# volume-em/empanada

Measured on AMD Instinct MI355X. Metric: Mvox/s end-to-end 3D panoptic inference (incl. consensus); PQ vs CPU ref, higher is better.
Workload: dtype f32

## Files before the change

### empanada_amd/_hip.py

```python
import ctypes
import os

import torch

_HERE = os.path.dirname(os.path.abspath(__file__))
LIB_PATH = os.path.join(_HERE, 'libemp_hip.so')

MAX_KS = 11
MAX_CLASSES = 16
MAX_CENTERS = 4096
CENTER_LIMIT = 65535


class HipError(RuntimeError):
    pass


_c = ctypes
_P = _c.c_void_p
_I = _c.c_int
_L = _c.c_int64
_F = _c.c_float
_U32 = _c.c_uint32

SIGNATURES = {
    'emp_version': (_I, []),
    'emp_last_error': (_c.c_char_p, []),
    'emp_device_count': (_I, []),
    'emp_bn_act_nhwc': (_I, [_P, _P, _P, _P, _I, _L, _I, _P, _L, _P]),
    'emp_dwconv_nhwc': (_I, [_P, _P, _P, _I, _I, _I, _I, _I, _P, _P]),
    'emp_upsample_bilinear': (_I, [_P, _I, _I, _I, _I, _P, _P, _I, _I, _P, _P]),
    'emp_conv_bn_act_proj_nhwc': (_I, [_P, _P, _P, _P, _I] + [_I] * 10 + [_P, _I, _P, _P, _L, _P]),
    'emp_conv_k_slab': (_I, [_L, _I, _I, _I]),
    'emp_conv_k_slab_cin': (_I, [_L, _I, _I, _I, _I]),
    'emp_conv_k_slab_geom': (_I, [_L, _I, _I, _I, _I, _I, _I, _I, _I]),
    'emp_conv1x1_ws_eligible': (_I, [_L, _I, _I, _I, _I, _I, _I, _I]),
    'emp_conv1x1_ws_kind_for': (_I, [_L, _I, _I, _I, _I, _I, _I, _I, _I]),
    'emp_conv1x1_ws_launches': (_L, [_I]),
    'emp_gconv_chunk': (_I, [_I]),
    'emp_gconv3x3_bn_act_nhwc': (_I, [_P, _L, _P, _P, _P, _I, _I, _I, _I, _I, _I, _I, _P, _L, _P]),
    'emp_conv_bn_act_nhwc': (_I, [_P, _P, _P, _P, _P, _L, _I] + [_I] * 10 + [_P, _L, _P]),
    'emp_conv_splitk_plan': (_I, [_L, _I, _I, _I, _I]),
    'emp_conv_splitk_bn_act_nhwc': (_I, [_P, _P, _P, _P, _P, _L, _I] + [_I] * 11 + [_P, _P, _L, _P]),
    'emp_wino_input_transform': (_I, [_P, _I, _I, _I, _I, _I, _P, _L, _P, _P]),
    'emp_gemm_nt_batched': (_I, [_P, _P, _I, _L, _I, _I, _P, _P]),
    'emp_wino4_input_transform': (_I, [_P, _I, _I, _I, _I, _I, _P, _L, _P, _P]),
    'emp_wino4_output_transform': (_I, [_P, _P, _L, _I, _I, _I, _I, _I, _P, _P, _I, _P, _L, _P]),
    'emp_wino4_conv_bn_act_nhwc': (_I, [_P, _I, _I, _I, _I, _I, _P, _L, _P, _I, _P, _P, _I, _P, _L, _P]),
    'emp_wino4_fused_eligible': (_I, [_L, _I, _I, _I]),
    'emp_wino3_input_transform': (_I, [_P, _I, _I, _I, _I, _I, _P, _L, _P, _P]),
    'emp_wino3_output_transform': (_I, [_P, _P, _L, _I, _I, _I, _I, _I, _P, _P, _I, _P, _L, _P]),
    'emp_wino_gemm_fused': (_I, [_P, _I, _I, _I, _I, _I, _P, _L, _P, _I, _P, _P]),
    'emp_wino_output_transform': (_I, [_P, _P, _L, _I, _I, _I, _I, _I, _P, _P, _I, _P, _L, _P]),
    'emp_chain_class': (_I, [_L, _P, _P, _P, _I, _P, _P, _P, _P, _L, _L, _c.c_double, _c.c_double, _P, _P, _P, _P]),
    'emp_lsap_maximize': (_L, [_P, _L, _L, _P, _P]),
    'emp_slices_to_input': (_I, [_P, _L, _L, _L, _I, _I, _I, _I, _I, _F, _F, _P, _P]),
    'emp_slices_to_input_scaled': (_I, [_P, _L, _L, _L] + [_I] * 7 + [_P, _P, _P, _P, _I, _F, _F, _P, _P]),
    'emp_pointwise_out_nhwc': (_I, [_P, _P, _P, _L, _L, _I, _I, _P, _P]),
    'emp_bn_relu_maxpool_nhwc': (_I, [_P, _P, _P, _I, _I, _I, _I, _P, _P]),
    'emp_stem_conv7_bn_relu_maxpool': (_I, [_P, _P, _P, _P, _I, _I, _I, _P, _P]),
    'emp_logits_to_prob': (_I, [_P, _I, _I, _L, _P, _P]),
    'emp_upsample_bilinear_prob': (_I, [_P, _I, _I, _I, _I, _P, _P, _I, _I, _P, _I, _P]),
    'emp_pr_upsample2x': (_I, [_P, _I, _I, _I, _I, _P, _P, _P]),
    'emp_pr_topk_work_bytes': (_L, [_I, _L]),
    'emp_pr_topk': (_I, [_P, _I, _L, _I, _P, _L, _P, _P]),
    'emp_pr_point_sample': (_I, [_P, _L, _P, _I, _I, _I, _I, _I, _P, _I, _I, _I, _P, _P, _I, _P]),
    'emp_pr_scatter': (_I, [_P, _I, _P, _I, _I, _I, _L, _P, _P]),
    'emp_median_harden_stack': (_I, [_P, _I, _I, _L, _I, _F, _P, _P, _P]),
    'emp_median_step': (_I, [_c.POINTER(_P), _I, _L, _P, _P]),
    'emp_harden': (_I, [_P, _I, _I, _L, _F, _P, _P]),
    'emp_find_centers': (_I, [_P, _I, _I, _I, _F, _I, _I, _P, _P, _P]),
    'emp_find_centers_work_elems': (_L, [_I, _I, _I, _I]),
    'emp_find_centers_ws': (_I, [_P, _I, _I, _I, _F, _I, _I, _P, _P, _P, _P]),
    'emp_group_work_elems': (_L, [_I, _I]),
    'emp_group_pixels': (_I, [_P, _P, _I, _P, _I, _I, _I, _I, _P, _U32, _P, _P, _P]),
    'emp_fuse_work_elems': (_L, [_I, _I, _I]),
    'emp_fuse_panoptic': (_I, [_P, _P, _I, _I, _I, _I, _I, _I, _U32, _L, _L, _L, _P, _P, _P, _P]),
    'emp_fuse_lut': (_I, [_P, _P, _I, _I, _I, _I, _I, _I, _U32, _L, _L, _P, _P]),
    'emp_fuse_apply': (_I, [_P, _P, _I, _I, _I, _I, _I, _I, _U32, _L, _L, _P, _P, _P, _P]),
    'emp_runs_count': (_I, [_P, _I, _I, _I, _P, _P]),
    'emp_scan_tmp_elems': (_L, [_L]),
    'emp_exclusive_scan_i32': (_I, [_P, _L, _P, _P, _P]),
    'emp_runs_extract': (_I, [_P, _I, _I, _I, _P, _P, _P, _P, _P]),
    'emp_runs_label_work_elems': (_L, [_L]),
    'emp_runs_label': (_I, [_P, _P, _P, _P, _L, _I, _I, _I, _L, _U32, _P, _P, _P, _P, _P, _P, _P, _P, _P]),
    'emp_runs_overlap_next': (_I, [_P, _P, _P, _P, _P, _L, _I, _I, _I, _L, _P, _L, _P, _P]),
    'emp_rle_decode': (_I, [_P, _P, _P, _L, _P, _P]),
    'emp_rle_encode_work_elems': (_L, [_L]),
    'emp_rle_encode': (_I, [_P, _L, _P, _P, _P, _P, _P]),
    'emp_box_pairs': (_I, [_P, _L, _P, _L, _I, _P, _P, _I, _P, _L, _P, _P]),
    'emp_rle_pair_intersections': (_I, [_P, _P, _P, _P, _L, _P, _P]),
    'emp_sort_work_bytes': (_L, [_L]),
    'emp_sort_u64_i32': (_I, [_P, _P, _P, _P, _L, _I, _I, _P, _L, _P]),
    'emp_vote_work_bytes': (_L, [_L]),
    'emp_vote_ranges': (_I, [_P, _P, _P, _L, _I, _I, _P, _L, _P, _P, _P]),
    'emp_fill_runs_u32': (_I, [_P, _L, _P, _P, _P, _L, _P, _P]),
    'emp_fill_table_u32': (_I, [_P, _L, _I, _I, _P, _P, _P, _P, _P, _L, _P]),
    'emp_scatter_yz_u32': (_I, [_P, _I, _I, _I, _P, _P, _P, _P, _P, _L, _P]),
    'emp_fill_runs_u8': (_I, [_P, _L, _P, _P, _L, _c.c_uint8, _P]),
    'emp_triplets_reduce_work_bytes': (_L, [_L]),
    'emp_triplets_reduce': (_I, [_P, _L, _P, _L, _P, _P, _P]),
    'emp_track_work_elems': (_L, [_L]),
    'emp_track_lift': (_I, [_I, _P, _P, _P, _P, _P, _L, _I, _I, _I, _I, _I, _L, _P, _P, _P, _P, _P]),
    'emp_track_lift_yz': (_I, [_P, _P, _P, _P, _L, _L, _I, _I, _I, _L, _P, _P, _P]),
    'emp_tile_lift': (_I, [_P, _P, _P, _P, _P, _L, _I, _I, _I, _I, _L, _P, _P, _P, _P, _P]),
    'emp_track_sort_work_bytes': (_L, [_L]),
    'emp_track_sort': (_I, [_P, _P, _L, _I, _P, _L, _P, _P, _P, _P, _P]),
    'emp_track_offsets': (_I, [_P, _L, _L, _P, _P]),
    'emp_track_expand': (_I, [_P, _P, _L, _L, _P, _P]),
    'emp_track_clip': (_I, [_P, _P, _L, _L, _L, _P, _P, _P, _P, _P]),
}

_lib = None


def load():
    global _lib
    if _lib is None:
        if not os.path.exists(LIB_PATH):
            raise HipError(f"{LIB_PATH} not found: build it with `python -m empanada_amd.build` "
                           "(hipcc --offload-arch=gfx950). There is no CPU fallback.")
        lib = ctypes.CDLL(LIB_PATH)
        for name, (res, args) in SIGNATURES.items():
            fn = getattr(lib, name)
            fn.restype = res
            fn.argtypes = args
        _lib = lib
    return _lib


def require_gpu():
    if torch.cuda._is_in_bad_fork():
# ... 695 lines not shown
    N, C, h, w = logits.shape
    assert logits.is_cuda and logits.dtype == torch.float32 and logits.is_contiguous()
    up = torch.empty((N, C, 2 * h, 2 * w), dtype=torch.float32, device=logits.device)
    unc = torch.empty((N, 4 * h * w), dtype=torch.float32, device=logits.device)
    call('emp_pr_upsample2x', logits.data_ptr(), N, C, h, w, up.data_ptr(), unc.data_ptr(), stream(),
         alg_bytes=4 * (logits.numel() + up.numel() + unc.numel()))
    return up, unc


def pr_topk(unc, k):
    require_gpu()
    N, HW = unc.shape
    assert unc.is_cuda and unc.dtype == torch.float32 and unc.is_contiguous() and 1 <= k <= HW
    wb = query('emp_pr_topk_work_bytes', N, HW)
    work = torch.empty((wb,), dtype=torch.uint8, device=unc.device)
    idx = torch.empty((N, k), dtype=torch.int32, device=unc.device)
    call('emp_pr_topk', unc.data_ptr(), N, HW, int(k), _ptr(work), wb, _ptr(idx), stream(), alg_bytes=4 * 6 * unc.numel())
    return idx


def pr_point_sample(features, coarse, idx, H, W, ld):
    require_gpu()
    N, CF, Hf, Wf = features.shape
    C = coarse.shape[1]
    assert features.is_cuda and features.dtype == torch.float32 and features.stride(1) == 1
    fps = features.stride(3)
    assert features.stride(2) == Wf * fps and features.stride(0) == Hf * Wf * fps, "NHWC features required"
    assert coarse.is_contiguous() and coarse.shape == (N, C, Hf, Wf) and idx.shape[0] == N and idx.dtype == torch.int32
    k = idx.shape[1]
    X0 = torch.empty((N * k, ld), dtype=torch.float32, device=features.device)
    X1 = torch.empty((N * k, ld), dtype=torch.float32, device=features.device)
    call('emp_pr_point_sample', features.data_ptr(), fps, coarse.data_ptr(), N, Hf, Wf, CF, C, _ptr(idx), k, int(H), int(W),
         X0.data_ptr(), X1.data_ptr(), int(ld), stream(), alg_bytes=4 * N * k * (4 * CF + 2 * ld))
    return X0, X1


def pr_scatter(points, idx, logits):
    require_gpu()
    N, C, H, W = logits.shape
    k = idx.shape[1]
    assert points.shape[0] == N * k and points.stride(1) == 1 and logits.is_contiguous()
    call('emp_pr_scatter', points.data_ptr(), points.stride(0), _ptr(idx), N, C, k, H * W, logits.data_ptr(), stream(),
         alg_bytes=8 * N * k * C)
    return logits


def as_pixels(mat, cols=None):
    P, ld = mat.shape
    v = mat.view(1, P, 1, ld).permute(0, 3, 1, 2)
    return v if cols is None else v[:, :cols]


def stem_conv7_bn_relu_maxpool(x, w_tc, scale, shift):
    require_gpu()
    N, C, H, W = x.shape
    assert C == 1 and x.is_cuda and x.dtype == torch.float32 and x.is_contiguous()
    assert tuple(w_tc.shape) == (49, 64) and w_tc.is_contiguous()
    OH, OW = (H - 1) // 2 + 1, (W - 1) // 2 + 1
    PH, PW = (OH - 1) // 2 + 1, (OW - 1) // 2 + 1
    y = torch.empty((N, 64, PH, PW), dtype=torch.float32, device=x.device, memory_format=torch.channels_last)
    call('emp_stem_conv7_bn_relu_maxpool', x.data_ptr(), _ptr(w_tc), _ptr(scale), _ptr(shift), N, H, W, y.data_ptr(),
         stream(), alg_bytes=4 * (x.numel() + y.numel()), alg_flops=2 * N * OH * OW * 64 * 49)
    return y


def wino4_filter_transform(w_oihw):
    g = w_oihw.detach().double().cpu()

    def comb(a, b, c):
        return [a / 4.0, -((a + b) + c) / 6.0, ((b - a) - c) / 6.0, (a / 24.0 + b / 12.0) + c / 6.0,
                (a / 24.0 - b / 12.0) + c / 6.0, c]

    rows = comb(g[:, :, 0, :], g[:, :, 1, :], g[:, :, 2, :])
    U = []
    for r in rows:
        U.extend(comb(r[:, :, 0], r[:, :, 1], r[:, :, 2]))
    return torch.stack(U, dim=0).float().contiguous()


def wino4_fused_eligible(T, Cin, Cout, has_scale_shift=True):
    return bool(load().emp_wino4_fused_eligible(int(T), int(Cin), int(Cout), int(bool(has_scale_shift))))


def wino4_conv_bn_act(x, U, tiles_dev, dil, scale=None, shift=None, relu=False, out=None, fused=None):
    require_gpu()
    N, Cin, H, W = x.shape
    Cout = U.shape[1]
    assert x.is_cuda and x.dtype == torch.float32 and x.is_contiguous(memory_format=torch.channels_last)
    T = tiles_dev.shape[0]
    if fused is None:
        fused = wino4_fused_eligible(T, Cin, Cout, scale is not None and shift is not None)
    if out is None:
        out = torch.empty((N, Cout, H, W), dtype=torch.float32, device=x.device, memory_format=torch.channels_last)
    assert out.shape == (N, Cout, H, W) and out.stride(1) == 1
    ops = out.stride(3)
    assert out.stride(2) == W * ops and out.stride(0) == H * W * ops, "NHWC channel slice required"
    st = stream()
    if fused:
        call('emp_wino4_conv_bn_act_nhwc', x.data_ptr(), N, H, W, Cin, dil, _ptr(tiles_dev), T, _ptr(U), Cout,
             _ptr(scale), _ptr(shift), int(bool(relu)), out.data_ptr(), ops, st, profile_as='emp_gemm_nt_batched',
             alg_bytes=4 * (x.numel() + U.numel() + N * Cout * H * W), alg_flops=2 * 36 * T * Cout * Cin)
        return out
    V = torch.empty((36, T, Cin), dtype=torch.float32, device=x.device)
    Mw = torch.empty((36, T, Cout), dtype=torch.float32, device=x.device)
    call('emp_wino4_input_transform', x.data_ptr(), N, H, W, Cin, dil, _ptr(tiles_dev), T, _ptr(V), st,
         alg_bytes=4 * (x.numel() + V.numel()))
    call('emp_gemm_nt_batched', _ptr(V), _ptr(U), 36, T, Cout, Cin, _ptr(Mw), st,
         alg_bytes=4 * (V.numel() + U.numel() + Mw.numel()), alg_flops=2 * 36 * T * Cout * Cin)
    call('emp_wino4_output_transform', _ptr(Mw), _ptr(tiles_dev), T, N, H, W, Cout, dil, _ptr(scale), _ptr(shift),
         int(bool(relu)), out.data_ptr(), ops, st, alg_bytes=4 * (Mw.numel() + N * Cout * H * W))
    return out


def conv_k_slab(M, Cout, batch=1, has_residual=False, Cin=None, geom=None, relu=False):
    if geom is not None:
        KH, KW, stride, pad = geom
        return int(load().emp_conv_k_slab_geom(int(M), int(Cout), int(bool(has_residual)), int(Cin), int(KH), int(KW),
                                               int(stride), int(pad), 2 if relu == 'gate' else int(bool(relu))))
    if Cin is not None:
        return int(load().emp_conv_k_slab_cin(int(M), int(Cout), int(batch), int(bool(has_residual)), int(Cin)))
    return int(load().emp_conv_k_slab(int(M), int(Cout), int(batch), int(bool(has_residual))))


_WINO3_G = [[0.5, 0.0, 0.0], [-0.5, -0.5, -0.5], [-1.0 / 6, 1.0 / 6, -1.0 / 6], [1.0 / 6, 1.0 / 3, 2.0 / 3], [0.0, 0.0, 1.0]]


def wino3_filter_transform(w_oihw):
    g = w_oihw.detach().double().cpu()

    def comb(a, b, c):
        return [(G[0] * a + G[1] * b) + G[2] * c for G in _WINO3_G]

    rows = comb(g[:, :, 0, :], g[:, :, 1, :], g[:, :, 2, :])
    U = []
    for r in rows:
        U.extend(comb(r[:, :, 0], r[:, :, 1], r[:, :, 2]))
    return torch.stack(U, dim=0).float().contiguous()


def wino3_conv_bn_act(x, U, tiles_dev, dil, scale=None, shift=None, relu=False, out=None):
    require_gpu()
    N, Cin, H, W = x.shape
    Cout = U.shape[1]
    assert x.is_cuda and x.dtype == torch.float32 and x.is_contiguous(memory_format=torch.channels_last)
    T = tiles_dev.shape[0]
    V = torch.empty((25, T, Cin), dtype=torch.float32, device=x.device)
    Mw = torch.empty((25, T, Cout), dtype=torch.float32, device=x.device)
    if out is None:
        out = torch.empty((N, Cout, H, W), dtype=torch.float32, device=x.device, memory_format=torch.channels_last)
    assert out.shape == (N, Cout, H, W) and out.stride(1) == 1
    ops = out.stride(3)
    assert out.stride(2) == W * ops and out.stride(0) == H * W * ops, "NHWC channel slice required"
    st = stream()
    call('emp_wino3_input_transform', x.data_ptr(), N, H, W, Cin, dil, _ptr(tiles_dev), T, _ptr(V), st,
         alg_bytes=4 * (x.numel() + V.numel()))
    call('emp_gemm_nt_batched', _ptr(V), _ptr(U), 25, T, Cout, Cin, _ptr(Mw), st,
         alg_bytes=4 * (V.numel() + U.numel() + Mw.numel()), alg_flops=2 * 25 * T * Cout * Cin)
    call('emp_wino3_output_transform', _ptr(Mw), _ptr(tiles_dev), T, N, H, W, Cout, dil, _ptr(scale), _ptr(shift),
         int(bool(relu)), out.data_ptr(), ops, st, alg_bytes=4 * (Mw.numel() + N * Cout * H * W))
    return out


def conv_bn_act_proj_nhwc(x, w_okkc, scale, shift, relu, proj_w, proj_b=None, stride=1, pad=0, dil=1, keep=False):
    require_gpu()
    N, Cin, H, W = x.shape
    Cout, KH, KW, _ = w_okkc.shape
# ... 15 lines not shown
```

### empanada_amd/csrc/emp_wino4.hip

```cpp
#include "emp_common.h"
#include "emp_wino4.h"
#include <stdlib.h>
#include <type_traits>

typedef float f32x4 __attribute__((ext_vector_type(4)));

#define WF_THREADS 512
#define WF_G 32
#define WF_S 16
#define WF_RS 34
#define WF_PS (WF_S * WF_RS)
#define WF_PF 3
#define WF_XCH (WF_THREADS * 48)
#define WF_T_MIN 3136

struct WfGeom {
    const float *x, *U, *scale, *shift;
    const int32_t *tiles;
    float *out;
    int64_t T, out_ps;
    int H, W, dil, groups;
};

template <int CIN, int COUT, bool RELU>
__global__ __launch_bounds__(WF_THREADS, 2) void wino4_fused_kernel(WfGeom g)
{
    constexpr int KS = CIN / WF_S;
    constexpr int CG = COUT / 64;
    __shared__ __attribute__((aligned(16))) float Vs[36 * WF_PS > WF_XCH ? 36 * WF_PS : WF_XCH];

    const int tid = threadIdx.x, wave = tid >> 6, lane = tid & 63;
    const int tl = tid >> 4, ch = tid & 15;
    const int ci = lane & 15, q = lane >> 4;
    const int odd = q >> 1;
    const int h = wave >> 2, w4 = wave & 3;

    const int xcd = blockIdx.x & 7, slot = blockIdx.x >> 3, per = gridDim.x >> 3;
    const int lo = (int)((int64_t)g.groups * xcd / 8), hi = (int)((int64_t)g.groups * (xcd + 1) / 8);
    const int n_items = slot < hi - lo ? ((hi - lo - slot + per - 1) / per) * CG : 0;

    auto load_raw = [&](int item, int s, v1 (&raw)[6][6]) -> int {
        const int64_t t = (int64_t)(lo + slot + (item / CG) * per) * WF_G + tl;
        const bool live = t < g.T;
        const int64_t tc = live ? t : g.T - 1;
        const int n = g.tiles[3 * tc], by = g.tiles[3 * tc + 1], bx = g.tiles[3 * tc + 2];
        const uint32_t src = 4u * ((uint32_t)n * (uint32_t)(g.H * g.W * CIN) + (uint32_t)(WF_S * s + ch));
        const char *xb = reinterpret_cast<const char *>(g.x);
        int mask = 0;
        uint32_t xo[6];
#pragma unroll
        for (int b = 0; b < 6; ++b) {
            const int xx = bx + b * g.dil;
            if (live && xx >= 0 && xx < g.W) mask |= 64 << b;
            xo[b] = 4u * (uint32_t)(min(max(xx, 0), g.W - 1) * CIN);
        }
#pragma unroll
        for (int a = 0; a < 6; ++a) {
            const int yy = by + a * g.dil;
            if (live && yy >= 0 && yy < g.H) mask |= 1 << a;
            const uint32_t row = src + 4u * (uint32_t)(min(max(yy, 0), g.H - 1) * (g.W * CIN));
#pragma unroll
            for (int b = 0; b < 6; ++b) raw[a][b] = {*reinterpret_cast<const float *>(xb + (row + xo[b]))};
        }
        return mask;
    };
    auto transform = [&](const v1 (&raw)[6][6], int mask) {
        v1 tt[6][6];
#pragma unroll
        for (int a = 0; a < 6; ++a) {
            v1 d[6];
#pragma unroll
            for (int b = 0; b < 6; ++b) d[b] = {(mask >> a & 1) && (mask >> (6 + b) & 1) ? raw[a][b].x : 0.f};
            wino4_bt(d, tt[a]);
        }
        float *dst = &Vs[ch * WF_RS + tl];
#pragma unroll
        for (int v = 0; v < 6; ++v) {
            v1 col[6], r[6];
#pragma unroll
            for (int a = 0; a < 6; ++a) col[a] = tt[a][v];
            wino4_bt(col, r);
#pragma unroll
            for (int u = 0; u < 6; ++u) dst[(u * 6 + v) * WF_PS] = r[u].x;
        }
    };

    const float *Al = &Vs[3 * h * WF_PS + (8 * (q & 1) + odd) * WF_RS + ci];
    const float *Ul = g.U + ((int64_t)3 * h * COUT + 16 * w4 + ci) * CIN + 8 * (q & 1) + 4 * odd;

    v1 raw[6][6];
    int mask = 0;
    if (n_items > 0) mask = load_raw(0, 0, raw);
    for (int item = 0; item < n_items; ++item) {
        const int cg = item % CG;
        f32x4 acc[18][2];
#pragma unroll
        for (int lp = 0; lp < 18; ++lp)
#pragma unroll
            for (int rt = 0; rt < 2; ++rt) acc[lp][rt] = {0.f, 0.f, 0.f, 0.f};

#pragma unroll 1
        for (int s = 0; s < KS; ++s) {
            transform(raw, mask);
            __syncthreads();
            const float *up = Ul + (int64_t)cg * 64 * CIN + WF_S * s;
            auto uoff = [](int lp) { return (int64_t)((lp / 3) * 6 + lp % 3) * COUT * CIN; };
            float4 bq[WF_PF];
#pragma unroll
            for (int lp = 0; lp < WF_PF; ++lp) bq[lp] = *reinterpret_cast<const float4 *>(up + uoff(lp));
            if (s + 1 < KS) mask = load_raw(item, s + 1, raw);
#pragma unroll
            for (int lp = 0; lp < 18; ++lp) {
                float4 c = bq[lp % WF_PF];
                asm volatile("" : "+v"(c.x), "+v"(c.y), "+v"(c.z), "+v"(c.w));
                if (lp + WF_PF < 18) bq[lp % WF_PF] = *reinterpret_cast<const float4 *>(up + uoff(lp + WF_PF));
                const auto s0 = __builtin_amdgcn_permlane32_swap(__float_as_uint(c.x), __float_as_uint(c.y), false, false);
                const auto s1 = __builtin_amdgcn_permlane32_swap(__float_as_uint(c.z), __float_as_uint(c.w), false, false);
                const float bv[4] = {__uint_as_float(s0[0]), __uint_as_float(s1[0]), __uint_as_float(s0[1]), __uint_as_float(s1[1])};
                const float *ap = Al + ((lp / 3) * 6 + lp % 3) * WF_PS;
#pragma unroll
                for (int j = 0; j < 4; ++j)
#pragma unroll
                    for (int rt = 0; rt < 2; ++rt)
                        acc[lp][rt] = __builtin_amdgcn_mfma_f32_16x16x4f32(ap[2 * j * WF_RS + 16 * rt], bv[j], acc[lp][rt], 0, 0, 0);
            }
            __syncthreads();
        }

        const int co = cg * 64 + 16 * w4 + ci;
        float keep[4][3][4];
        float *xw = &Vs[((wave ^ 4) * 48) * 64 + lane];
        const float *xr = &Vs[(wave * 48) * 64 + lane];
        auto rows = [&](auto rtc, auto sendc) {
            constexpr int rt = decltype(rtc)::value;
            constexpr bool send = decltype(sendc)::value;
#pragma unroll
            for (int bb = 0; bb < 3; ++bb)
#pragma unroll
                for (int r = 0; r < 4; ++r) {
                    v1 m[6], rr[4];
#pragma unroll
                    for (int a = 0; a < 6; ++a) m[a] = {acc[3 * a + bb][rt][r]};
                    wino4_at(m, rr);
#pragma unroll
                    for (int a = 0; a < 4; ++a) {
                        if (send) xw[((r * 3 + bb) * 4 + a) * 64] = rr[a].x;
                        else keep[r][bb][a] = rr[a].x;
                    }
                }
        };
        using std::integral_constant;
        if (h == 0) {
            rows(integral_constant<int, 1>(), integral_constant<bool, true>());
            rows(integral_constant<int, 0>(), integral_constant<bool, false>());
        } else {
            rows(integral_constant<int, 0>(), integral_constant<bool, true>());
            rows(integral_constant<int, 1>(), integral_constant<bool, false>());
        }
        if (item + 1 < n_items) mask = load_raw(item + 1, 0, raw);
        __syncthreads();

        const float sc = g.scale[co], sh = g.shift[co];
        const int64_t t0 = (int64_t)(lo + slot + (item / CG) * per) * WF_G + 16 * h + 4 * q;
#pragma unroll
        for (int r = 0; r < 4; ++r) {
            const int64_t t = t0 + r;
            if (t < g.T) {
                const int n = g.tiles[3 * t], oy = g.tiles[3 * t + 1] + g.dil, ox = g.tiles[3 * t + 2] + g.dil;
                float *dst = g.out + (int64_t)n * g.H * g.W * g.out_ps + co;
#pragma unroll
                for (int a = 0; a < 4; ++a) {
                    v1 sm[6], yv[4];
#pragma unroll
                    for (int bb = 0; bb < 3; ++bb) {
                        const float got = xr[((r * 3 + bb) * 4 + a) * 64];
                        sm[bb] = {h ? got : keep[r][bb][a]};
                        sm[3 + bb] = {h ? keep[r][bb][a] : got};
                    }
                    wino4_at(sm, yv);
#pragma unroll
                    for (int b = 0; b < 4; ++b) {
                        const int yy = oy + a * g.dil, xx = ox + b * g.dil;
                        if (yy < g.H && xx < g.W) {
                            float v = __fadd_rn(__fmul_rn(yv[b].x, sc), sh);
                            if (RELU) v = fmaxf(v, 0.f);
                            dst[((int64_t)yy * g.W + xx) * g.out_ps] = v;
                        }
                    }
                }
            }
        }
        __syncthreads();
    }
}

static bool wf_off()
{
    static const char *off = getenv("EMP_WINO4_NO_FUSED");
    return off && off[0] == '1';
}

static bool wf_shape_ok(int64_t T, int Cin, int Cout)
{
    return ((Cin == 64 && Cout == 64) || (Cin == 128 && Cout == 128)) && T > 0 && 16 * T * Cin < (1LL << 30) &&
           emp_conv_k_slab(T, Cout, 36, 0) == WF_S;
}

extern "C" int emp_wino4_fused_eligible(int64_t T, int Cin, int Cout, int has_scale_shift)
{
    if (wf_off() || !has_scale_shift) return 0;
    if (!(Cin == 64 && Cout == 64)) return 0;
    return wf_shape_ok(T, Cin, Cout) && T >= WF_T_MIN;
}

extern "C" int emp_wino4_conv_bn_act_nhwc(const float *x, int N, int H, int W, int Cin, int dil, const int32_t *tiles,
                                          int64_t T, const float *U, int Cout, const float *scale, const float *shift,
                                          int relu, float *out, int64_t out_pixel_stride, void *stream)
{
    EMP_REQUIRE(x && tiles && U && scale && shift && out, "wino4_conv: null pointer (scale and shift are required)");
    EMP_REQUIRE(N > 0 && H > 0 && W > 0 && dil >= 1 && T >= 0, "wino4_conv: bad shape");
    if (out_pixel_stride == 0) out_pixel_stride = Cout;
    EMP_REQUIRE(out_pixel_stride >= Cout, "wino4_conv: bad pixel stride");
    EMP_REQUIRE(((reinterpret_cast<uintptr_t>(x) | reinterpret_cast<uintptr_t>(U)) & 15) == 0 &&
                (reinterpret_cast<uintptr_t>(out) & 3) == 0, "wino4_conv: alignment");
    if (T == 0) return EMP_OK;
    EMP_REQUIRE(wf_shape_ok(T, Cin, Cout), "wino4_conv: 64 -> 64 or 128 -> 128 with the K-slab 16 plan only (T = %lld, %d -> %d)",
                (long long)T, Cin, Cout);
    EMP_REQUIRE((int64_t)N * H * W * Cin < (1LL << 30) && T < (1LL << 31) - WF_G, "wino4_conv: activation too large for 32-bit byte offsets");
    WfGeom g;
    g.x = x; g.U = U; g.scale = scale; g.shift = shift; g.tiles = tiles; g.out = out;
    g.T = T; g.out_ps = out_pixel_stride; g.H = H; g.W = W; g.dil = dil;
    g.groups = (int)emp_cdiv(T, WF_G);
    hipStream_t st = emp_stream(stream);
    const dim3 grid(256), block(WF_THREADS);
    if (Cin == 64) {
        if (relu) hipLaunchKernelGGL((wino4_fused_kernel<64, 64, true>), grid, block, 0, st, g);
        else hipLaunchKernelGGL((wino4_fused_kernel<64, 64, false>), grid, block, 0, st, g);
    } else {
        if (relu) hipLaunchKernelGGL((wino4_fused_kernel<128, 128, true>), grid, block, 0, st, g);
        else hipLaunchKernelGGL((wino4_fused_kernel<128, 128, false>), grid, block, 0, st, g);
    }
    EMP_CHECK_LAUNCH("emp_wino4_conv_bn_act_nhwc");
    return EMP_OK;
}
```

### empanada_amd/models/panoptic_deeplab.py

```python
import zlib
from typing import List

import torch
import torch.nn as nn
import torch.nn.functional as F

__all__ = ['PanopticDeepLab', 'PanopticDeepLabPR', 'PointRendSemSegHead', 'resnet_encoder', 'prepare_for_inference',
           'tune_fused_convs',
           'synthesize_weights']

_RESNETS = {
    'resnet18': ('basic', [2, 2, 2, 2]), 'resnet34': ('basic', [3, 4, 6, 3]),
    'resnet50': ('bottleneck', [3, 4, 6, 3]), 'resnet101': ('bottleneck', [3, 4, 23, 3]),
    'resnet152': ('bottleneck', [3, 8, 36, 3]),
}


def _conv_bn_act(nin, nout, k, stride=1, groups=1, act=True):
    layers = [nn.Conv2d(nin, nout, k, stride=stride, padding=(k - 1) // 2, groups=groups, bias=False),
              nn.BatchNorm2d(nout)]
    if act:
        layers.append(nn.ReLU(inplace=True))
    return nn.Sequential(*layers)

# ... 105 lines not shown

    def candidates(self, has_residual, shape=None):
        c = self.conv
        out = ['miopen']
        square = (c.bias is None and c.padding_mode == 'zeros' and c.kernel_size[0] == c.kernel_size[1]
                  and c.stride[0] == c.stride[1] and c.padding[0] == c.padding[1] and c.dilation[0] == c.dilation[1]
                  and c.weight.dtype == torch.float32)
        if square and c.groups == 1 and c.in_channels % 16 == 0:
            out.append('direct')
            if shape is not None and c.in_channels % 32 == 0 and c.out_channels % 4 == 0 and self.bn.relu in (0, 1, False, True):
                from .. import _hip
                k, st, pd, dl = c.kernel_size[0], c.stride[0], c.padding[0], c.dilation[0]
                oh = (shape[2] + 2 * pd - dl * (k - 1) - 1) // st + 1
                ow = (shape[3] + 2 * pd - dl * (k - 1) - 1) // st + 1
                if _hip.conv_splitk_plan(shape[0] * oh * ow, c.out_channels, c.in_channels, k, k) > 1:
                    out.append('direct_sk')
            if (c.kernel_size == (3, 3) and c.stride == (1, 1) and c.padding == c.dilation and c.out_channels % 4 == 0
                    and c.in_channels % 32 == 0 and not has_residual):
                out.extend(['wino', 'wino_sep', 'wino4', 'wino3'])
        gw = c.in_channels // c.groups
        if (square and c.groups > 1 and c.in_channels == c.out_channels and c.kernel_size == (3, 3) and c.padding == (1, 1)
                and c.dilation == (1, 1) and c.stride[0] in (1, 2) and gw % 8 == 0 and 8 <= gw <= 128 and not has_residual):
            out.append('grouped')
        return out

    def _prepare(self, impl):
        from .. import _hip
        if impl in ('direct', 'direct_sk', 'grouped') and self._w_okkc is None:
            self._w_okkc = self.conv.weight.detach().permute(0, 2, 3, 1).contiguous()
        if impl in ('wino', 'wino_sep') and self._U is None:
            self._U = _hip.wino_filter_transform(self.conv.weight.detach())
        if impl == 'wino4' and self._U4 is None:
            self._U4 = _hip.wino4_filter_transform(self.conv.weight.detach()).to(self.conv.weight.device)
        if impl == 'wino3' and self._U3 is None:
            self._U3 = _hip.wino3_filter_transform(self.conv.weight.detach()).to(self.conv.weight.device)

    def release(self, keep):
        if keep not in ('direct', 'direct_sk', 'grouped'):
            self._w_okkc = None
        if keep not in ('wino', 'wino_sep'):
            self._U = None
        if keep != 'wino4':
            self._U4 = None
        if keep != 'wino3':
            self._U3 = None
        if keep not in ('wino', 'wino_sep', 'wino4', 'wino3'):
            self._tiles = {}

    def forward(self, x, residual=None, out=None):
        self._seen = (tuple(x.shape), residual is not None)
        impl = self.impl
        if impl == 'miopen' or not (x.is_cuda and x.dtype == torch.float32):
            return self.bn(self.conv(x), residual, out)
        from .. import _hip
        c = self.conv
        if not x.is_contiguous(memory_format=torch.channels_last):
            x = x.contiguous(memory_format=torch.channels_last)
        self._prepare(impl)
        if impl in ('direct', 'direct_sk'):
            if residual is not None and not residual.is_contiguous(memory_format=torch.channels_last):
                residual = residual.contiguous(memory_format=torch.channels_last)
            if impl == 'direct_sk':
                oh = (x.shape[2] + 2 * c.padding[0] - c.dilation[0] * (c.kernel_size[0] - 1) - 1) // c.stride[0] + 1
                ow = (x.shape[3] + 2 * c.padding[0] - c.dilation[0] * (c.kernel_size[0] - 1) - 1) // c.stride[0] + 1
                ks = _hip.conv_splitk_plan(x.shape[0] * oh * ow, c.out_channels, c.in_channels, *c.kernel_size)
                if ks > 1:
                    return _hip.conv_splitk_bn_act_nhwc(x, self._w_okkc, self.bn.scale, self.bn.shift, residual,
                                                        self.bn.relu, c.stride[0], c.padding[0], c.dilation[0], out,
                                                        k_splits=ks)
            return _hip.conv_bn_act_nhwc(x, self._w_okkc, self.bn.scale, self.bn.shift, residual, self.bn.relu,
                                         c.stride[0], c.padding[0], c.dilation[0], out)
        assert residual is None
        if impl == 'grouped':
            return _hip.gconv3x3_bn_act_nhwc(x, self._w_okkc, c.groups, self.bn.scale, self.bn.shift, self.bn.relu,
                                             c.stride[0], out)
        m = {'wino4': 4, 'wino3': 3}.get(impl, 2)
        key = (x.shape[0], x.shape[2], x.shape[3], m)
        if key not in self._tiles:
            self._tiles[key] = torch.from_numpy(_hip.wino_tiles(key[0], key[1], key[2], c.dilation[0], m)).to(x.device)
        if impl == 'wino3':
            return _hip.wino3_conv_bn_act(x, self._U3, self._tiles[key], c.dilation[0], self.bn.scale, self.bn.shift,
                                          self.bn.relu, out)
        if impl == 'wino4':
            return _hip.wino4_conv_bn_act(x, self._U4, self._tiles[key], c.dilation[0], self.bn.scale, self.bn.shift,
                                          self.bn.relu, out)
        return _hip.wino_conv_bn_act(x, self._U, self._tiles[key], c.dilation[0], self.bn.scale, self.bn.shift,
                                     self.bn.relu, out, fused=(impl == 'wino'))


def _up_bilinear(x, size, hip_ops, out=None):
    if hip_ops and x.is_cuda and x.dtype == torch.float32:
        from .. import _hip
        return _hip.upsample_bilinear(x, size, out=out)
    y = F.interpolate(x, size=size, mode='bilinear', align_corners=True)
    if out is not None:
        out.copy_(y)
        return out
    return y


def _conv_bn_into(seq, x, out):
    if isinstance(seq[0], FusedConvBNAct):
        seq[0](x, out=out)
    else:
        seq[1](seq[0](x), out=out)
    for extra in list(seq)[2:]:
        assert isinstance(extra, (nn.Identity, nn.Dropout)), "unexpected module after the fused epilogue"


def _can_write_into(seq, x):
    if not (isinstance(seq, nn.Sequential) and len(seq) >= 2 and x.is_cuda and x.dtype == torch.float32):
        return False
    return isinstance(seq[0], FusedConvBNAct) or (isinstance(seq[0], nn.Conv2d) and isinstance(seq[1], FusedBNAct))


class _Basic(nn.Module):
    expansion = 1

    def __init__(self, inplanes, planes, stride=1, downsample=None, dilation=1):
        super().__init__()
        self.conv1 = nn.Conv2d(inplanes, planes, 3, stride, 1, bias=False)
        self.bn1 = nn.BatchNorm2d(planes)
        self.relu = nn.ReLU(inplace=True)
        self.conv2 = nn.Conv2d(planes, planes, 3, 1, 1, bias=False)
        self.bn2 = nn.BatchNorm2d(planes)
        self.downsample = downsample

    def forward(self, x):
        idt = x if self.downsample is None else self.downsample(x)
        if isinstance(self.conv1, FusedConvBNAct):
            return self.conv2(self.conv1(x), idt)
        if isinstance(self.bn1, FusedBNAct):
            out = self.bn1(self.conv1(x))
            return self.bn2(self.conv2(out), idt)
        out = self.relu(self.bn1(self.conv1(x)))
        out = self.bn2(self.conv2(out))
        return self.relu(out + idt)


class _Bottleneck(nn.Module):
    expansion = 4

    def __init__(self, inplanes, planes, stride=1, downsample=None, dilation=1):
        super().__init__()
        self.conv1 = nn.Conv2d(inplanes, planes, 1, bias=False)
        self.bn1 = nn.BatchNorm2d(planes)
        self.conv2 = nn.Conv2d(planes, planes, 3, stride, padding=dilation, dilation=dilation, bias=False)
        self.bn2 = nn.BatchNorm2d(planes)
        self.conv3 = nn.Conv2d(planes, planes * 4, 1, bias=False)
        self.bn3 = nn.BatchNorm2d(planes * 4)
        self.relu = nn.ReLU(inplace=True)
        self.downsample = downsample

    def forward(self, x):
        idt = x if self.downsample is None else self.downsample(x)
        if isinstance(self.conv1, FusedConvBNAct):
            return self.conv3(self.conv2(self.conv1(x)), idt)
        if isinstance(self.bn1, FusedBNAct):
            out = self.bn2(self.conv2(self.bn1(self.conv1(x))))
            return self.bn3(self.conv3(out), idt)
        out = self.relu(self.bn1(self.conv1(x)))
        out = self.relu(self.bn2(self.conv2(out)))
        out = self.bn3(self.conv3(out))
        return self.relu(out + idt)


class _Cfg:
    def __init__(self):
# ... 482 lines not shown
```

### include/emp_hip.h

```cpp
#ifndef EMP_HIP_H
#define EMP_HIP_H

#include <stdint.h>

#ifdef __cplusplus
extern "C" {
#endif

#define EMP_OK 0
#define EMP_EINVAL (-1)
#define EMP_ELAUNCH (-2)
#define EMP_ENODEV (-3)

#define EMP_MAX_KS 11
#define EMP_MAX_CLASSES 16
#define EMP_MAX_CENTERS 4096
#define EMP_CENTER_LIMIT 65535

int emp_version(void);
const char *emp_last_error(void);
int emp_device_count(void);

int emp_slices_to_input(const uint8_t *vol, int64_t stride_slice, int64_t stride_row, int64_t stride_col,
                        int n_slices, int h, int w, int hp, int wp, float mean255, float inv_std255,
                        float *out, void *stream);

int emp_slices_to_input_scaled(const uint8_t *vol, int64_t stride_slice, int64_t stride_row, int64_t stride_col,
                               int n_slices, int h, int w, int dh, int dw, int hp, int wp, const int32_t *row_off,
                               const int16_t *row_coef, const int32_t *col_off, const int16_t *col_coef, int area,
                               float mean255, float inv_std255, float *out, void *stream);

int emp_bn_act_nhwc(const float *x, const float *scale, const float *shift, const float *residual,
                    int relu, int64_t n_pixels, int C, float *out, int64_t out_pixel_stride, void *stream);

int emp_dwconv_nhwc(const float *x, const float *w_kkc, const float *bias, int N, int H, int W, int C,
                    int k, float *y, void *stream);

int emp_upsample_bilinear(const float *x, int N, int C, int h, int w, const int64_t *x_strides,
                          float *y, int H, int W, const int64_t *y_strides, void *stream);

int emp_conv_k_slab(int64_t M, int Cout, int batch, int has_residual);
int emp_conv_k_slab_cin(int64_t M, int Cout, int batch, int has_residual, int Cin);
int emp_conv_k_slab_geom(int64_t M, int Cout, int has_residual, int Cin, int KH, int KW, int stride, int pad, int relu);
int emp_conv1x1_ws_eligible(int64_t M, int Cin, int Cout, int KH, int KW, int stride, int pad, int relu);
int emp_conv1x1_ws_kind_for(int64_t M, int Cin, int Cout, int KH, int KW, int stride, int pad, int relu, int has_residual);
int64_t emp_conv1x1_ws_launches(int kind);
int emp_conv_bn_act_nhwc(const float *x, const float *w_okkc, const float *scale, const float *shift,
                         const float *residual, int64_t res_pixel_stride, int relu, int N, int H, int W,
                         int Cin, int Cout, int KH, int KW, int stride, int pad, int dil, float *out,
                         int64_t out_pixel_stride, void *stream);
int emp_conv_splitk_plan(int64_t M, int Cout, int Cin, int KH, int KW);
int emp_conv_splitk_bn_act_nhwc(const float *x, const float *w_okkc, const float *scale, const float *shift,
                                const float *residual, int64_t res_pixel_stride, int relu, int N, int H, int W,
                                int Cin, int Cout, int KH, int KW, int stride, int pad, int dil, int k_splits,
                                float *work, float *out, int64_t out_pixel_stride, void *stream);

int emp_conv_bn_act_proj_nhwc(const float *x, const float *w_okkc, const float *scale, const float *shift,
                              int relu, int N, int H, int W, int Cin, int Cout, int KH, int KW, int stride,
                              int pad, int dil, const float *proj_w, int proj_n, float *proj_out,
                              float *out, int64_t out_pixel_stride, void *stream);

int emp_gconv_chunk(int group_w);
int emp_gconv3x3_bn_act_nhwc(const float *x, int64_t x_pixel_stride, const float *w_okkc, const float *scale,
                             const float *shift, int relu, int N, int H, int W, int groups, int group_w,
                             int stride, float *out, int64_t out_pixel_stride, void *stream);

int emp_wino_input_transform(const float *x, int N, int H, int W, int C, int dil, const int32_t *tiles,
                             int64_t T, float *V, void *stream);
int emp_gemm_nt_batched(const float *A, const float *B, int batch, int64_t M, int N, int K, float *C,
                        void *stream);
int emp_wino_gemm_fused(const float *x, int N, int H, int W, int Cin, int dil, const int32_t *tiles,
                        int64_t T, const float *U, int Cout, float *Mw, void *stream);
int emp_wino_output_transform(const float *Mw, const int32_t *tiles, int64_t T, int N, int H, int W,
                              int Cout, int dil, const float *scale, const float *shift, int relu,
                              float *out, int64_t out_pixel_stride, void *stream);

int emp_wino4_input_transform(const float *x, int N, int H, int W, int C, int dil, const int32_t *tiles,
                              int64_t T, float *V, void *stream);
int emp_wino4_output_transform(const float *Mw, const int32_t *tiles, int64_t T, int N, int H, int W,
                               int Cout, int dil, const float *scale, const float *shift, int relu,
                               float *out, int64_t out_pixel_stride, void *stream);
int emp_wino4_conv_bn_act_nhwc(const float *x, int N, int H, int W, int Cin, int dil, const int32_t *tiles, int64_t T,
                               const float *U, int Cout, const float *scale, const float *shift, int relu,
                               float *out, int64_t out_pixel_stride, void *stream);
int emp_wino4_fused_eligible(int64_t T, int Cin, int Cout, int has_scale_shift);

int emp_wino3_input_transform(const float *x, int N, int H, int W, int C, int dil, const int32_t *tiles,
                              int64_t T, float *V, void *stream);
int emp_wino3_output_transform(const float *Mw, const int32_t *tiles, int64_t T, int N, int H, int W,
                               int Cout, int dil, const float *scale, const float *shift, int relu,
                               float *out, int64_t out_pixel_stride, void *stream);

int emp_pointwise_out_nhwc(const float *x, const float *w, const float *bias, int64_t n_pixels,
                           int64_t pixels_per_image, int C, int Cout, float *out, void *stream);

int emp_bn_relu_maxpool_nhwc(const float *x, const float *scale, const float *shift, int N, int H, int W,
                             int C, float *y, void *stream);

int emp_stem_conv7_bn_relu_maxpool(const float *x, const float *w_tc, const float *scale, const float *shift,
                                   int N, int H, int W, float *y, void *stream);

int emp_logits_to_prob(const float *logits, int N, int C, int64_t HW, float *prob, void *stream);

int emp_upsample_bilinear_prob(const float *x, int N, int C, int h, int w, const int64_t *x_strides,
                               float *y, int H, int W, const int64_t *y_strides, int prob, void *stream);

int emp_median_harden_stack(const float *prob, int D, int C, int64_t HW, int ks, float thr,
                            uint8_t *out_sem, float *out_prob, void *stream);

int emp_median_step(const float *const *slices_host, int ks, int64_t n, float *out, void *stream);

int emp_harden(const float *prob, int D, int C, int64_t HW, float thr, uint8_t *out_sem,
               void *stream);

int emp_find_centers(const float *hmp, int D, int h, int w, float thr, int k, int cap,
                     int32_t *out_idx, int32_t *out_count, void *stream);

int64_t emp_find_centers_work_elems(int D, int h, int w, int cap);
int emp_find_centers_ws(const float *hmp, int D, int h, int w, float thr, int k, int cap, int32_t *work,
                        int32_t *out_idx, int32_t *out_count, void *stream);

int64_t emp_group_work_elems(int D, int cap);
int emp_group_pixels(const int32_t *ctr_idx, const int32_t *ctr_count, int cap,
                     const float *offsets, int D, int h, int w, int step, const uint8_t *sem,
                     uint32_t thing_mask, float *work, uint16_t *out_ids, void *stream);

int64_t emp_fuse_work_elems(int D, int cap, int n_classes);
int emp_fuse_panoptic(const uint8_t *sem, const uint16_t *ids, int D, int H, int W, int up,
                      int cap, int n_classes, uint32_t thing_mask, int64_t label_divisor,
                      int64_t stuff_area, int64_t void_label, int32_t *work,
                      uint32_t *out_pan_u32, int64_t *out_pan_i64, void *stream);
int emp_fuse_lut(const uint8_t *sem, const uint16_t *ids, int D, int H, int W, int up, int cap,
                 int n_classes, uint32_t thing_mask, int64_t label_divisor, int64_t stuff_area,
                 int32_t *work, void *stream);
int emp_fuse_apply(const uint8_t *sem, const uint16_t *ids, int D, int H, int W, int up, int cap,
                   int n_classes, uint32_t thing_mask, int64_t label_divisor, int64_t void_label,
                   const int32_t *work, uint32_t *out_pan_u32, int64_t *out_pan_i64, void *stream);

int emp_runs_count(const uint32_t *pan, int D, int H, int W, int32_t *row_counts, void *stream);
int64_t emp_scan_tmp_elems(int64_t n);
int emp_exclusive_scan_i32(const int32_t *in, int64_t n, int32_t *out, int32_t *tmp, void *stream);
int emp_runs_extract(const uint32_t *pan, int D, int H, int W, const int32_t *row_offsets,
                     int32_t *r_start, int32_t *r_len, uint32_t *r_val, void *stream);
int64_t emp_runs_label_work_elems(int64_t n_runs);
int emp_runs_label(const int32_t *r_start, const int32_t *r_len, const uint32_t *r_val,
                   const int32_t *row_offsets, int64_t n_runs, int D, int H, int W,
                   int64_t label_divisor, uint32_t cc_mask, int32_t *work, int32_t *r_comp,
                   int32_t *c_slice, int64_t *c_label, int64_t *c_area, int32_t *c_box,
                   int32_t *c_first, int32_t *n_comp_out, void *stream);

int emp_runs_overlap_next(const int32_t *r_start, const int32_t *r_len, const int32_t *r_comp,
                          const uint32_t *r_val, const int32_t *row_offsets, int64_t n_runs, int D,
                          int H, int W, int64_t label_divisor, int32_t *out_triplets,
                          int64_t cap_triplets, int32_t *n_out, void *stream);

int emp_rle_decode(const int64_t *starts, const int64_t *runs, const int64_t *offsets, int64_t n_runs,
                   int64_t *out_indices, void *stream);
int64_t emp_rle_encode_work_elems(int64_t n);
int emp_rle_encode(const int64_t *indices, int64_t n, int32_t *work, int64_t *out_starts,
                   int64_t *out_runs, int32_t *n_runs_out, void *stream);

int emp_box_pairs(const int32_t *boxes_a, int64_t na, const int32_t *boxes_b, int64_t nb, int ndim,
                  const int32_t *src_a, const int32_t *src_b, int upper_only, int32_t *out_pairs,
                  int64_t cap, int32_t *n_out, void *stream);

int emp_rle_pair_intersections(const int64_t *starts, const int64_t *lens, const int64_t *inst_off,
                               const int32_t *pairs, int64_t n_pairs, int64_t *out_inter,
                               void *stream);
// ... 71 lines not shown
```

Before: 134.0.

## Double-buffer wino4 fused kernel LDS and enable it for 128-channel convs

The fused Winograd F(4,3) kernel now keeps two LDS buffers for the transformed input. The two half-block wave groups stagger their loads and transforms so that only one barrier is needed per K-step instead of two. A-operand LDS reads are software-prefetched a few MFMAs ahead using sched barriers, and lane-derived indices are recomputed to reduce register pressure. A new site-eligibility function also forces the fused path for 128x128-channel convolutions with large tile counts, which extends the kernel to a new shape and risks correctness or occupancy problems there.

```diff
diff --git a/empanada_amd/_hip.py b/empanada_amd/_hip.py
--- a/empanada_amd/_hip.py
+++ b/empanada_amd/_hip.py
@@ -48,6 +48,7 @@
     'emp_wino4_output_transform': (_I, [_P, _P, _L, _I, _I, _I, _I, _I, _P, _P, _I, _P, _L, _P]),
     'emp_wino4_conv_bn_act_nhwc': (_I, [_P, _I, _I, _I, _I, _I, _P, _L, _P, _I, _P, _P, _I, _P, _L, _P]),
     'emp_wino4_fused_eligible': (_I, [_L, _I, _I, _I]),
+    'emp_wino4_fused_site': (_I, [_L, _I, _I, _I]),
     'emp_wino3_input_transform': (_I, [_P, _I, _I, _I, _I, _I, _P, _L, _P, _P]),
     'emp_wino3_output_transform': (_I, [_P, _P, _L, _I, _I, _I, _I, _I, _P, _P, _I, _P, _L, _P]),
     'emp_wino_gemm_fused': (_I, [_P, _I, _I, _I, _I, _I, _P, _L, _P, _I, _P, _P]),
@@ -909,6 +910,10 @@
     return bool(load().emp_wino4_fused_eligible(int(T), int(Cin), int(Cout), int(bool(has_scale_shift))))
 
 
+def wino4_fused_site(T, Cin, Cout, has_scale_shift=True):
+    return bool(load().emp_wino4_fused_site(int(T), int(Cin), int(Cout), int(bool(has_scale_shift))))
+
+
 def wino4_conv_bn_act(x, U, tiles_dev, dil, scale=None, shift=None, relu=False, out=None, fused=None):
     require_gpu()
     N, Cin, H, W = x.shape
diff --git a/empanada_amd/csrc/emp_wino4.hip b/empanada_amd/csrc/emp_wino4.hip
--- a/empanada_amd/csrc/emp_wino4.hip
+++ b/empanada_amd/csrc/emp_wino4.hip
@@ -11,8 +11,11 @@
 #define WF_RS 34
 #define WF_PS (WF_S * WF_RS)
 #define WF_PF 3
+#define WF_AD 3
+#define WF_BUF (36 * WF_PS)
 #define WF_XCH (WF_THREADS * 48)
 #define WF_T_MIN 3136
+#define WF_T_MIN_128 8192
 
 struct WfGeom {
     const float *x, *U, *scale, *shift;
@@ -27,19 +30,19 @@
 {
     constexpr int KS = CIN / WF_S;
     constexpr int CG = COUT / 64;
-    __shared__ __attribute__((aligned(16))) float Vs[36 * WF_PS > WF_XCH ? 36 * WF_PS : WF_XCH];
-
-    const int tid = threadIdx.x, wave = tid >> 6, lane = tid & 63;
-    const int tl = tid >> 4, ch = tid & 15;
-    const int ci = lane & 15, q = lane >> 4;
-    const int odd = q >> 1;
+    static_assert(2 * WF_BUF >= WF_XCH && KS % 2 == 0, "the exchange area overlays the ring; an item ends in buffer 1");
+    __shared__ __attribute__((aligned(16))) float Vs[2 * WF_BUF];
+
+    const int tid = threadIdx.x, wave = __builtin_amdgcn_readfirstlane(tid >> 6);
     const int h = wave >> 2, w4 = wave & 3;
+    auto tid_again = [&]() { int t = tid; asm volatile("" : "+v"(t)); return t; };
 
     const int xcd = blockIdx.x & 7, slot = blockIdx.x >> 3, per = gridDim.x >> 3;
     const int lo = (int)((int64_t)g.groups * xcd / 8), hi = (int)((int64_t)g.groups * (xcd + 1) / 8);
     const int n_items = slot < hi - lo ? ((hi - lo - slot + per - 1) / per) * CG : 0;
 
     auto load_raw = [&](int item, int s, v1 (&raw)[6][6]) -> int {
+        const int tt_ = tid_again(), tl = tt_ >> 4, ch = tt_ & 15;
         const int64_t t = (int64_t)(lo + slot + (item / CG) * per) * WF_G + tl;
         const bool live = t < g.T;
         const int64_t tc = live ? t : g.T - 1;
@@ -64,7 +67,7 @@
         }
         return mask;
     };
-    auto transform = [&](const v1 (&raw)[6][6], int mask) {
+    auto transform = [&](const v1 (&raw)[6][6], int mask, int buf) {
         v1 tt[6][6];
 #pragma unroll
         for (int a = 0; a < 6; ++a) {
@@ -73,7 +76,8 @@
             for (int b = 0; b < 6; ++b) d[b] = {(mask >> a & 1) && (mask >> (6 + b) & 1) ? raw[a][b].x : 0.f};
             wino4_bt(d, tt[a]);
         }
-        float *dst = &Vs[ch * WF_RS + tl];
+        const int tt_ = tid_again();
+        float *dst = &Vs[buf * WF_BUF + (tt_ & 15) * WF_RS + (tt_ >> 4)];
 #pragma unroll
         for (int v = 0; v < 6; ++v) {
             v1 col[6], r[6];
@@ -85,8 +89,8 @@
         }
     };
 
-    const float *Al = &Vs[3 * h * WF_PS + (8 * (q & 1) + odd) * WF_RS + ci];
-    const float *Ul = g.U + ((int64_t)3 * h * COUT + 16 * w4 + ci) * CIN + 8 * (q & 1) + 4 * odd;
+    auto a_lane = [&]() { const int l = tid_again() & 63; return &Vs[3 * h * WF_PS + (8 * ((l >> 4) & 1) + (l >> 5)) * WF_RS + (l & 15)]; };
+    auto u_lane = [&]() { const int l = tid_again() & 63; return g.U + ((3 * h * COUT + 16 * w4 + (l & 15)) * CIN + 8 * ((l >> 4) & 1) + 4 * (l >> 5)); };
 
     v1 raw[6][6];
     int mask = 0;
@@ -99,16 +103,27 @@
 #pragma unroll
             for (int rt = 0; rt < 2; ++rt) acc[lp][rt] = {0.f, 0.f, 0.f, 0.f};
 
+        transform(raw, mask, 0);
+        if (h) mask = load_raw(item, 1, raw);
+        __syncthreads();
+        if (h) transform(raw, mask, 1);
 #pragma unroll 1
         for (int s = 0; s < KS; ++s) {
-            transform(raw, mask);
-            __syncthreads();
-            const float *up = Ul + (int64_t)cg * 64 * CIN + WF_S * s;
+            const int nxt = s + 1 + h;
+            const float *up = u_lane() + cg * 64 * CIN + WF_S * s;
             auto uoff = [](int lp) { return (int64_t)((lp / 3) * 6 + lp % 3) * COUT * CIN; };
             float4 bq[WF_PF];
 #pragma unroll
             for (int lp = 0; lp < WF_PF; ++lp) bq[lp] = *reinterpret_cast<const float4 *>(up + uoff(lp));
-            if (s + 1 < KS) mask = load_raw(item, s + 1, raw);
+            if (nxt < KS) mask = load_raw(item, nxt, raw);
+            const float *Ab = a_lane() + (s & 1) * WF_BUF;
+            auto a_ld = [&](int k) {
+                const float *p = Ab + ((k / 12) * 6 + (k / 4) % 3) * WF_PS + 2 * (k % 4) * WF_RS;
+                return float2{p[0], p[16]};
+            };
+            float2 ar[WF_AD + 1];
+#pragma unroll
+            for (int k = 0; k < WF_AD; ++k) ar[k] = a_ld(k);
 #pragma unroll
             for (int lp = 0; lp < 18; ++lp) {
                 float4 c = bq[lp % WF_PF];
@@ -117,20 +132,26 @@
                 const auto s0 = __builtin_amdgcn_permlane32_swap(__float_as_uint(c.x), __float_as_uint(c.y), false, false);
                 const auto s1 = __builtin_amdgcn_permlane32_swap(__float_as_uint(c.z), __float_as_uint(c.w), false, false);
                 const float bv[4] = {__uint_as_float(s0[0]), __uint_as_float(s1[0]), __uint_as_float(s0[1]), __uint_as_float(s1[1])};
-                const float *ap = Al + ((lp / 3) * 6 + lp % 3) * WF_PS;
-#pragma unroll
-                for (int j = 0; j < 4; ++j)
-#pragma unroll
-                    for (int rt = 0; rt < 2; ++rt)
-                        acc[lp][rt] = __builtin_amdgcn_mfma_f32_16x16x4f32(ap[2 * j * WF_RS + 16 * rt], bv[j], acc[lp][rt], 0, 0, 0);
+#pragma unroll
+                for (int j = 0; j < 4; ++j) {
+                    const int k = 4 * lp + j;
+                    if (k + WF_AD < 72) ar[(k + WF_AD) % (WF_AD + 1)] = a_ld(k + WF_AD);
+                    __builtin_amdgcn_sched_barrier(0);
+                    acc[lp][0] = __builtin_amdgcn_mfma_f32_16x16x4f32(ar[k % (WF_AD + 1)].x, bv[j], acc[lp][0], 0, 0, 0);
+                    acc[lp][1] = __builtin_amdgcn_mfma_f32_16x16x4f32(ar[k % (WF_AD + 1)].y, bv[j], acc[lp][1], 0, 0, 0);
+                    __builtin_amdgcn_sched_barrier(0);
+                }
             }
-            __syncthreads();
-        }
-
-        const int co = cg * 64 + 16 * w4 + ci;
+            if (h) __syncthreads();
+            if (nxt < KS) transform(raw, mask, nxt & 1);
+            if (!h) __syncthreads();
+        }
+
+        const int le = tid_again() & 63, cie = le & 15, qe = le >> 4;
+        const int co = cg * 64 + 16 * w4 + cie;
         float keep[4][3][4];
-        float *xw = &Vs[((wave ^ 4) * 48) * 64 + lane];
-        const float *xr = &Vs[(wave * 48) * 64 + lane];
+        float *xw = &Vs[((wave ^ 4) * 48) * 64 + le];
+        const float *xr = &Vs[(wave * 48) * 64 + le];
         auto rows = [&](auto rtc, auto sendc) {
             constexpr int rt = decltype(rtc)::value;
             constexpr bool send = decltype(sendc)::value;
@@ -161,7 +182,7 @@
         __syncthreads();
 
         const float sc = g.scale[co], sh = g.shift[co];
-        const int64_t t0 = (int64_t)(lo + slot + (item / CG) * per) * WF_G + 16 * h + 4 * q;
+        const int64_t t0 = (int64_t)(lo + slot + (item / CG) * per) * WF_G + 16 * h + 4 * qe;
 #pragma unroll
         for (int r = 0; r < 4; ++r) {
             const int64_t t = t0 + r;
@@ -211,6 +232,12 @@
     if (wf_off() || !has_scale_shift) return 0;
     if (!(Cin == 64 && Cout == 64)) return 0;
     return wf_shape_ok(T, Cin, Cout) && T >= WF_T_MIN;
+}
+
+extern "C" int emp_wino4_fused_site(int64_t T, int Cin, int Cout, int has_scale_shift)
+{
+    if (Cin == 128 && Cout == 128) return !wf_off() && has_scale_shift && wf_shape_ok(T, Cin, Cout) && T >= WF_T_MIN_128;
+    return emp_wino4_fused_eligible(T, Cin, Cout, has_scale_shift);
 }
 
 extern "C" int emp_wino4_conv_bn_act_nhwc(const float *x, int N, int H, int W, int Cin, int dil, const int32_t *tiles,
diff --git a/empanada_amd/models/panoptic_deeplab.py b/empanada_amd/models/panoptic_deeplab.py
--- a/empanada_amd/models/panoptic_deeplab.py
+++ b/empanada_amd/models/panoptic_deeplab.py
@@ -211,8 +211,10 @@
             return _hip.wino3_conv_bn_act(x, self._U3, self._tiles[key], c.dilation[0], self.bn.scale, self.bn.shift,
                                           self.bn.relu, out)
         if impl == 'wino4':
+            site = _hip.wino4_fused_site(self._tiles[key].shape[0], c.in_channels, c.out_channels,
+                                         self.bn.scale is not None and self.bn.shift is not None)
             return _hip.wino4_conv_bn_act(x, self._U4, self._tiles[key], c.dilation[0], self.bn.scale, self.bn.shift,
-                                          self.bn.relu, out)
+                                          self.bn.relu, out, fused=True if site else None)
         return _hip.wino_conv_bn_act(x, self._U, self._tiles[key], c.dilation[0], self.bn.scale, self.bn.shift,
                                      self.bn.relu, out, fused=(impl == 'wino'))
 
diff --git a/include/emp_hip.h b/include/emp_hip.h
--- a/include/emp_hip.h
+++ b/include/emp_hip.h
@@ -84,6 +84,7 @@
                                const float *U, int Cout, const float *scale, const float *shift, int relu,
                                float *out, int64_t out_pixel_stride, void *stream);
 int emp_wino4_fused_eligible(int64_t T, int Cin, int Cout, int has_scale_shift);
+int emp_wino4_fused_site(int64_t T, int Cin, int Cout, int has_scale_shift);
 
 int emp_wino3_input_transform(const float *x, int N, int H, int W, int C, int dil, const int32_t *tiles,
                               int64_t T, float *V, void *stream);
```

Result: no change. 134.6, median of 4 (+0.5%).
